# akshilpatel/tile-match-gym

Measured on AMD Instinct MI355X. Metric: env-steps/sec (whole node), 65536×10×10 boards, at 1/2/4/8 MI355X, higher is better.
Workload: dtype int8; 1 GPU; c2: 65536 x 10x10 boards per GPU, 4 colours, no specials, num_moves=30, autoreset, 3 episode-phase blocks offset by 10 steps, the timed window opening on a block's reset step (phases + 4); boards_per_gpu=65536, rows=10, cols=10, colours=4, env_groups_per_gpu=3, phase_blocks=3, policy=uniform, api=raw, graph=False, parallelism=dp1 (independent env shards, no collective)

## Files before the change

### tile-match-gym_amd/csrc/tmg_board.hip

```cpp
#include <hip/hip_runtime.h>
#include <stdint.h>

#include "pcg64.h"

namespace tmg {

#define WSYNC() __syncthreads()

#ifndef TMG_LEAN128_WAVES
#define TMG_LEAN128_WAVES 8
#endif
constexpr int kLean128Waves = TMG_LEAN128_WAVES;
constexpr int kLean128GenericWaves = 7;
constexpr int kGen128Waves = 5;
#ifndef TMG_RESET512_WAVES
#define TMG_RESET512_WAVES 8
#endif
#ifndef TMG_RESET128_WAVES
#define TMG_RESET128_WAVES 8
#endif
constexpr int kReset512Waves = TMG_RESET512_WAVES;
constexpr int kReset128Waves = TMG_RESET128_WAVES;
constexpr int kC5StepWaves = 4;

#define WFENCE() __builtin_amdgcn_fence(__ATOMIC_SEQ_CST, "wavefront")

#ifndef TMG_SMEM_DECL
#define TMG_SMEM_DECL(name) extern __shared__ __align__(16) unsigned char name[]
#endif

enum : int { SP_COOKIE = 1, SP_VLASER = 2, SP_HLASER = 4, SP_BOMB = 8 };
enum : int { M_NORMAL = 0, M_VLASER = 1, M_HLASER = 2, M_BOMB = 3, M_COOKIE = 4 };
enum : int { FL_DONE = 1, FL_COMBO = 2, FL_SHUF = 4, FL_RESET = 8, FL_OVF = 0x40, FL_ERR = 0x80 };
enum : int { TIER_MAIN = 0, TIER_SPILL = 2 };
enum : uint32_t { ST_INTERNAL = 1, ST_OVERFLOW = 2, ST_CALLER = 4 };

constexpr int kMaxShuffles = 1 << 12;

constexpr int kSpillWaves = 16;
struct SpillQ {
    uint32_t count, done;
    unsigned long long total;
    int64_t cap;
    int64_t env[1];
};

#ifndef TMG_COVER
#define TMG_COVER 0
#endif
enum : int {
    CV_SB_LEAN = 0,
    CV_SB_NORMAL,
    CV_SB_LASER,
    CV_SB_PERP_BOMB,
    CV_SB_ROW_BOMB,
    CV_SB_CLOSURE,
    CV_SB_FALLBACK,
    CV_LDS_NORMAL,
    CV_LDS_LASER,
    CV_LDS_BOMB,
    CV_LDS_FALLBACK,
    CV_SERIAL_STEP,
    CV_SERIAL_ACT,
    CV_SERIAL_COOKIE,
    CV_COMBO,
    CV_SPILL,
    CV_SPILL_RUN,
    CV_SHUFFLE,
    CV_REJECT,
    CV_FAST,
    CV_SHUFFLE_GEN,
    CV_REJECT_GEN,
    CV_RP_PASSES,
    CV_RP_PERP,
    CV_RP_VLONG,
    CV_RP_WIDE,
    CV_RP_REJECT,
    CV_COUNT = 32
};
#if TMG_COVER
#define COVER(site)                                                                                     \
    do {                                                                                                \
        if (lane == 0 && P.cover) atomicAdd(P.cover + (site), 1ULL);                                   \
    } while (0)
#define COVER_L0(site)                                                                                  \
    do {                                                                                                \
        if (P.cover) atomicAdd(P.cover + (site), 1ULL);                                                \
    } while (0)
#else
#define COVER(site) ((void)0)
#define COVER_L0(site) ((void)0)
#endif

struct Params {
    int R, C, N, A, W, k, smask, num_moves;
    uint32_t thr;
    uint32_t cmag, cm1mag;
    const uint64_t *jump;
    uint64_t sb_nl[2];
    uint64_t sb_nf[2];
    uint64_t sb_h[2];
    uint64_t sb_z;
    uint64_t sb_in[2], sb_u[2], sb_v[2];
    const uint64_t *sb_rows;
    uint32_t *status;
    void *oh;
    int oh_dtype, oh_ch, oh_nsel;
    uint32_t oh_sel;
    SpillQ *spill;
    void *spill_ws;
    unsigned long long *cover;
    uint8_t *vo_term;
    uint8_t *vo_mask;
    int64_t *vo_left;
    int8_t *vo_final;
    int32_t *vo_obs;
    int sample;
    int32_t pol_t;
    int64_t pol_first;
    uint64_t pol_key;
};

#ifndef TMG_KERNARG_PARAMS
#if defined(__HIP_DEVICE_COMPILE__)
#define TMG_KERNARG_PARAMS(p) (*(const Params *)__builtin_amdgcn_kernarg_segment_ptr())
#else
#define TMG_KERNARG_PARAMS(p) (p)
#endif
#endif

inline void build_sb_rows(int R, int C, uint64_t *tab) {
    for (int r = 0; r < R; r++) {
        uint64_t m[4] = {0, 0, 0, 0};
        for (int p = 0; p < (r + 1) * C && p < 128; p++) {
            if (p >= r * C) m[p & 1] |= 1ULL << (p >> 1);
            m[2 + (p & 1)] |= 1ULL << (p >> 1);
        }
        for (int i = 0; i < 4; i++) tab[r * 4 + i] = m[i];
    }
}

inline Params make_params(int R, int C, int k, int smask, int num_moves, const uint64_t *jump) {
    Params P;
    P.R = R; P.C = C; P.N = R * C;
    P.A = 2 * R * C - R - C;
    P.W = (P.A + 63) / 64;
    P.k = k; P.smask = smask; P.num_moves = num_moves;
    const uint32_t rng = (uint32_t)(k - 1), excl = rng + 1;
    P.thr = rng ? (UINT32_MAX - rng) % excl : 0u;
    P.cmag = ((1u << 20) + (uint32_t)C - 1) / (uint32_t)C;
    P.cm1mag = C > 1 ? ((1u << 20) + (uint32_t)C - 2) / (uint32_t)(C - 1) : 0u;
    P.jump = jump;
    for (int w = 0; w < 2; w++) P.sb_nl[w] = P.sb_nf[w] = P.sb_h[w] = P.sb_in[w] = P.sb_u[w] = P.sb_v[w] = 0;
    P.sb_z = 0;
    P.sb_rows = nullptr;
    P.status = nullptr;
    P.spill = nullptr;
    P.spill_ws = nullptr;
    P.cover = nullptr;
    P.oh = nullptr;
    P.oh_dtype = P.oh_ch = P.oh_nsel = 0;
    P.oh_sel = 0;
    P.vo_term = nullptr;
    P.vo_mask = nullptr;
    P.vo_left = nullptr;
    P.vo_final = nullptr;
    P.vo_obs = nullptr;
    P.sample = 0;
    P.pol_t = 0;
    P.pol_first = 0;
    P.pol_key = 0;
    if (P.N <= 128) {
        for (int p = 0; p < P.N; p++) {
            const int c = p % C, w = p & 1, b = p >> 1;
            P.sb_in[w] |= 1ULL << b;
            if (p >= C) P.sb_u[w] |= 1ULL << b;
            if (p >= 2 * C) P.sb_v[w] |= 1ULL << b;
            if (c <= C - 2) P.sb_nl[w] |= 1ULL << b;
            if (c >= 1) P.sb_nf[w] |= 1ULL << b;
            if (c <= C - 3) P.sb_h[w] |= 1ULL << b;
        }
        const int stride = (C & 1) ? C : C / 2;
        for (int b = 0; b < 64; b += stride) P.sb_z |= 1ULL << b;
    }
    return P;
}

__device__ __forceinline__ int div_c(const Params &P, int x) { return (int)(((uint32_t)x * P.cmag) >> 20); }
__device__ __forceinline__ int div_cm1(const Params &P, int x) { return (int)(((uint32_t)x * P.cm1mag) >> 20); }


__device__ __forceinline__ int64_t wg_env() {
    const int64_t per = gridDim.x >> 3;
    return (int64_t)(blockIdx.x & 7) * per + (blockIdx.x >> 3);
}

enum : int { SC_NACT = 0, SC_NNEW, SC_ERR, SC_NZ, SC_A, SC_B, SC_C, SC_D, SC_COUNT = 16 };

template <int MAXN_>
struct WsCore {
    static constexpr int MAXN = MAXN_;
    static constexpr int NP = MAXN / 64;
    static constexpr int MAXW = (2 * MAXN) / 64 + 2;
    uint64_t effw[MAXW];
    int32_t sc[SC_COUNT];
    static constexpr int PRE = MAXW * 8 + SC_COUNT * 4;
    int8_t lpad[PRE >= 128 ? 1 : 128 - PRE];
    alignas(4) int8_t brd[2 * MAXN];
    uint8_t mark[MAXN];
    alignas(8) int8_t trash[4 * 64];
    union alignas(16) {
        uint32_t draw[MAXN + 128];
        struct { int8_t tmp[2 * MAXN]; int16_t perm[MAXN]; } sh;
    } u;
};

template <int POOL_, int MLINES_, int MQ_, int MM_, int MPOOL_, int MSTK_>
struct ListStore {
    static constexpr int POOL = POOL_;
    static constexpr int MLINES = MLINES_;
    static constexpr int MQ = MQ_;
    static constexpr int MM = MM_;
    static constexpr int MPOOL = MPOOL_;
    static constexpr int MSTK = MSTK_;
    static constexpr int MV = 96;
    int16_t pool[POOL];
    int16_t ls[MLINES], ll[MLINES];
    int16_t q[MQ];
    int16_t mpool[MPOOL];
    int16_t ms[MM], mlen[MM];
    int8_t mname[MM], mcol[MM];
    int16_t fcell[MSTK], fidx[MSTK];
    int8_t ftype[MSTK], faux[MSTK];
    int16_t valid[MV];
    int16_t taken[MM], qpos[MM];
    int8_t qname[MM], qcol[MM];
    int32_t counts[16];
    int16_t pick[4];
};

constexpr int kCap128 = 64;
constexpr int kCap512 = 80;
template <int MAXN, int CAP = (MAXN > 128 ? kCap512 : kCap128)>
using WsSerial = ListStore<4 * CAP + 256, CAP + 64, 2 * CAP + 64, CAP + 32, 4 * CAP + 256, CAP + 8>;

template <int MAXN, int POOLB = 5 * MAXN + 3 * 64 + 64, int LINESB = 2 * MAXN + 2 * 64 + POOLB / 5 + 16>
using WsSerialBig = ListStore<POOLB, LINESB, LINESB, LINESB, POOLB + 3 * LINESB, MAXN + 8>;

template <int MAXN, bool GEN>
struct Ws : WsCore<MAXN> {};
template <int MAXN>
struct Ws<MAXN, true> : WsCore<MAXN> {
    WsSerial<MAXN> s;
};

__device__ __forceinline__ uint32_t umin(uint32_t a, uint32_t b) { return a < b ? a : b; }
__device__ __forceinline__ uint32_t umin3(uint32_t a, uint32_t b, uint32_t c) { return umin(umin(a, b), c); }
__device__ __forceinline__ uint32_t ne(int a, int b) { return (uint32_t)(a ^ b); }

__device__ __forceinline__ int wave_max(int v) {
    const int lo = (int)0x80000000;
    v = max(v, __builtin_amdgcn_update_dpp(lo, v, 0x111, 0xf, 0xf, false));
    v = max(v, __builtin_amdgcn_update_dpp(lo, v, 0x112, 0xf, 0xf, false));
    v = max(v, __builtin_amdgcn_update_dpp(lo, v, 0x114, 0xf, 0xf, false));
    v = max(v, __builtin_amdgcn_update_dpp(lo, v, 0x118, 0xf, 0xf, false));
    v = max(v, __builtin_amdgcn_update_dpp(lo, v, 0x142, 0xa, 0xf, false));
    v = max(v, __builtin_amdgcn_update_dpp(lo, v, 0x143, 0xc, 0xf, false));
    return __builtin_amdgcn_readlane(v, 63);
}

__device__ __forceinline__ int popc_below(uint64_t m) {
    return (int)__builtin_amdgcn_mbcnt_hi((uint32_t)(m >> 32), __builtin_amdgcn_mbcnt_lo((uint32_t)m, 0u));
}
#ifndef TMG_OPAQUE_V
#define TMG_OPAQUE_V(x) asm volatile("" : "+v"(x))
#endif
#ifndef TMG_KEEP_V
#define TMG_KEEP_V(x) asm volatile("" ::"v"(x))
// ... 133 lines not shown
struct Cells {
    uint32_t pk[NP];
    __device__ __forceinline__ int key(int i) const { return (int)(pk[i] & 0x7fffu); }
    __device__ __forceinline__ int r(int i) const { return (int)((pk[i] >> 9) & 63u); }
    __device__ __forceinline__ int c(int i) const { return 255 - (int)((pk[i] >> 1) & 255u); }
    __device__ __forceinline__ uint32_t vbad(int i) const { return (pk[i] >> 15) & 1u; }
    __device__ __forceinline__ uint32_t hbad(int i) const { return (pk[i] >> 16) & 1u; }
};
template <int NP>
__device__ __forceinline__ Cells<NP> make_cells(const Params &P, int lane) {
    Cells<NP> cl;
#pragma unroll
    for (int i = 0; i < NP; i++) {
        const int p = i * 64 + lane;
        const int r = div_c(P, p), c = p - r * P.C;
        const uint32_t vbad = (p < P.N && r >= 2) ? 0u : 1u;
        const uint32_t hbad = (p < P.N && c + 2 < P.C) ? 0u : 1u;
        cl.pk[i] = ((uint32_t)(((r & 63) << 8) | (255 - (c & 255))) << 1) | (vbad << 15) | (hbad << 16);
    }
    return cl;
}

template <class WS>
__device__ __forceinline__ void load_board(const Params &P, WS &w, int lane, const int8_t *src) {
    const int nb = 2 * P.N;
    if ((nb & 3) == 0) {
        const uint32_t *s = reinterpret_cast<const uint32_t *>(src);
        uint32_t *d = reinterpret_cast<uint32_t *>(w.brd);
        for (int i = lane; i < (nb >> 2); i += 64) d[i] = s[i];
    } else {
        for (int i = lane; i < nb; i += 64) w.brd[i] = src[i];
    }
}
template <class WS>
__device__ __forceinline__ void store_board(const Params &P, const WS &w, int lane, int8_t *dst) {
    const int nb = 2 * P.N;
    if ((nb & 3) == 0) {
        uint32_t *d = reinterpret_cast<uint32_t *>(dst);
        const uint32_t *s = reinterpret_cast<const uint32_t *>(w.brd);
        for (int i = lane; i < (nb >> 2); i += 64) d[i] = s[i];
    } else {
        for (int i = lane; i < nb; i += 64) dst[i] = w.brd[i];
    }
}

template <class WS>
__device__ __forceinline__ void store_onehot(const Params &P, const WS &w, int lane, int64_t e) {
    const int N = P.N, k = P.k, ch = P.oh_ch;
    const bool bytes = P.oh_dtype == 1;
    const uint32_t one = P.oh_dtype == 0 ? 0x3f800000u : 1u;
    uint8_t *o8 = reinterpret_cast<uint8_t *>(P.oh) + e * (int64_t)ch * N;
    uint32_t *o32 = reinterpret_cast<uint32_t *>(P.oh) + e * (int64_t)ch * N;
    for (int p = lane; p < N; p += 64) {
        const int x = w.brd[p], y = w.brd[N + p];
        for (int c = 0; c < ch; c++) {
            const bool on = c < k ? x == c + 1 : y == (int)(int8_t)(P.oh_sel >> (8 * (c - k)));
            if (bytes) o8[c * N + p] = on ? 1 : 0;
            else o32[c * N + p] = on ? one : 0u;
        }
    }
}

template <class WS>
__device__ __forceinline__ void store_mask(const Params &P, const WS &w, int lane, int64_t e, bool zero) {
    const int A = P.A;
    uint8_t *m = P.vo_mask + e * (int64_t)A;
    if ((A & 3) == 0) {
        uint32_t *m4 = reinterpret_cast<uint32_t *>(m);
        for (int i = lane; i < (A >> 2); i += 64) {
            const uint32_t b = zero ? 0u : (uint32_t)(w.effw[i >> 4] >> ((4 * i) & 63)) & 0xFu;
            m4[i] = (b * 0x00204081u) & 0x01010101u;
        }
    } else {
        for (int i = lane; i < A; i += 64) m[i] = zero ? (uint8_t)0 : (uint8_t)((w.effw[i >> 6] >> (i & 63)) & 1ULL);
    }
}

template <class WS>
__device__ __forceinline__ void store_obs(const Params &P, const WS &w, int lane, int64_t e) {
    int32_t *o = P.vo_obs + e * 2 * (int64_t)P.N;
    for (int p = lane; p < 2 * P.N; p += 64) o[p] = w.brd[p];
}

__device__ __forceinline__ void store_vo(const Params &P, int64_t e, int flags, int tnew) {
    if (P.vo_term) {
        const uint32_t v = ((flags & FL_DONE) ? 1u : 0u) | ((flags & FL_COMBO) ? 1u << 8 : 0u) |
                           ((flags & FL_SHUF) ? 1u << 16 : 0u) |
                           ((flags & (FL_ERR | FL_OVF)) ? 1u << 24 : 0u);
        reinterpret_cast<uint32_t *>(P.vo_term)[e] = v;
    }
    if (P.vo_left) P.vo_left[e] = (int64_t)(P.num_moves - tnew);
}

__host__ __device__ __forceinline__ uint64_t splitmix64(uint64_t x) {
    x += 0x9E3779B97F4A7C15ULL;
    x = (x ^ (x >> 30)) * 0xBF58476D1CE4E5B9ULL;
    x = (x ^ (x >> 27)) * 0x94D049BB133111EBULL;
    return x ^ (x >> 31);
}
__host__ __device__ __forceinline__ uint64_t policy_draw(uint64_t key, uint64_t gid, int32_t t) {
    const uint64_t base = splitmix64(key * 0xD1B54A32D192ED03ULL + gid);
    return splitmix64(base ^ ((uint64_t)t * 0x9E3779B97F4A7C15ULL)) >> 32;
}

__device__ __forceinline__ int sample_action(const Params &P, uint64_t effrow, int64_t e, int lane) {
#ifndef TMG_DRAW_VALU
#define TMG_DRAW_VALU 0
#endif
#if TMG_DRAW_VALU
    uint64_t gid = (uint64_t)(P.pol_first + e);
    TMG_OPAQUE_V(gid);
    const uint32_t h = (uint32_t)__builtin_amdgcn_readfirstlane((int)(uint32_t)policy_draw(P.pol_key, gid, P.pol_t));
#else
#ifndef TMG_KO
#define TMG_KO 0
#endif
    const uint32_t h = (TMG_KO & 2) ? (uint32_t)(e * 2654435761u) : (uint32_t)policy_draw(P.pol_key, (uint64_t)(P.pol_first + e), P.pol_t);
#endif
    const int W = P.W;
    const int pc = __popcll(effrow);
    int count = 0;
    for (int j = 0; j < W; j++) count += __builtin_amdgcn_readlane(pc, j);
    if (count == 0) return (int)(((uint64_t)h * (uint64_t)P.A) >> 32);
    int r = (int)(((uint64_t)h * (uint64_t)count) >> 32);
    int j = 0;
    for (; j < W - 1; j++) {
        const int c = __builtin_amdgcn_readlane(pc, j);
        if (r < c) break;
        r -= c;
    }
    const uint64_t x = rdlane64(effrow, j);
    const bool hit = ((x >> lane) & 1ULL) && popc_below(x) == r;
    return j * 64 + __ffsll((unsigned long long)__ballot(hit)) - 1;
}

__device__ __forceinline__ int nth_set_bit(uint64_t x, int r) {
    int pos = 0;
#pragma unroll
    for (int sh = 32; sh > 0; sh >>= 1) {
        const int c = __popcll(x & ((1ULL << sh) - 1ULL));
        const bool up = r >= c;
        r -= up ? c : 0;
        x = up ? x >> sh : x;
        pos += up ? sh : 0;
    }
    return pos;
}
__device__ __forceinline__ int32_t draw_row(const uint64_t *m, int W, int A, uint64_t h) {
    int count = 0;
    for (int j = 0; j < W; j++) count += __popcll(m[j]);
    if (count == 0) return (int32_t)((h * (uint64_t)A) >> 32);
    int r = (int)((h * (uint64_t)count) >> 32);
    int j = 0;
    uint64_t x = m[0];
    for (int c = __popcll(x); r >= c && j < W - 1; c = __popcll(x)) {
        r -= c;
        x = m[++j];
    }
    return j * 64 + nth_set_bit(x, r);
}

__device__ __forceinline__ bool eff_exact(const Params &P, const int8_t *brd, int a) {
    const int R = P.R, C = P.C, N = P.N;
    int r1, c1, r2, c2;
    action_coords(R, C, a, r1, c1, r2, c2);
    const int8_t *col = brd, *typ = brd + N;
    const int p = r1 * C + c1, q = r2 * C + c2;
    const int tp = typ[p], tq = typ[q];
    if ((tp != 0 && tp != 1) && (tq != 0 && tq != 1)) return true;
    if (tp < 0 || tq < 0) return true;
    const int cp = col[p], cq = col[q];
    auto CO = [&](int x) -> int { return x == p ? cq : (x == q ? cp : (int)col[x]); };
    auto TY = [&](int x) -> int { return x == p ? tq : (x == q ? tp : (int)typ[x]); };
    int rmin = (r1 < r2 ? r1 : r2) - 2; if (rmin < 0) rmin = 0;
// ... 1462 lines not shown
                if (r < 0) break;
                if (r > 0) { elim += r; iters++; lim = P.R - 1; continue; }
                COVER(CV_SB_FALLBACK);
            }
        }
        Det<MAXN / 64> d;
        const int rs = detect(P, w, lane, cells(), d, lim);
        if (rs < 0) break;
        lim = P.R - 1;
        if (fast) {
            COVER(CV_FAST);
            elim += fast_clear(P, w, lane, cells(), d, rs);
            lim = min(P.R - 1, rs + 2);
        } else {
            if constexpr (GEN && SBNB == 0) {
                uint64_t cols = 0;
                int rows = 0;
                const int r = plain ? simple_step_lds(P, w, lane, d, rs, cols, rows) : 0;
                if (r > 0) {
                    elim += r;
                    gravity(P, w, lane, cols);
                    WSYNC();
                    refill(P, w, lane, J, g, rows);
                    iters++;
                    lim = min(P.R - 1, rs + 2);
                    continue;
                }
                if (plain) COVER(CV_LDS_FALLBACK);
            }
            if constexpr (GEN) {
                int nz = count_colour_nonzero(P, w, lane);
                COVER(CV_SERIAL_STEP);
                if (lane == 0) {
                    w.sc[SC_NZ] = nz;
                    Serial<MAXN, L> S(P, w, *lists);
                    S.build_lines(rs);
                    if (!S.ovf) S.process_lines();
                    if (!S.ovf) S.resolve();
                    w.sc[SC_A] = S.ovf;
                }
                WSYNC();
                ovf |= w.sc[SC_A] != 0;
                elim += count_type_zero(P, w, lane);
            }
        }
        gravity(P, w, lane);
        WSYNC();
        refill(P, w, lane, J, g);
        iters++;
    }
    (void)iters;
    nn = w.sc[SC_NNEW];
    na = w.sc[SC_NACT];
    elim += nn;
    if (ovf) flags |= FL_OVF;
    if (err || w.sc[SC_ERR]) flags |= FL_ERR;
    flags |= ensure_playable(P, w, lane, J, g, cells(), !ovf && !err && !w.sc[SC_ERR]);
    return elim;
}

__device__ __forceinline__ LaneJump load_jump(const Params &P, int lane, const Rng &g) {
    const uint64_t *t = P.jump + lane * 4;
    LaneJump J;
    J.Aj = U128{t[0], t[1]};
    J.Gj = U128{t[2], t[3]};
    J.incG = mul128(U128{g.ilo, g.ihi}, J.Gj);
    return J;
}

__device__ __forceinline__ Rng load_rng(const uint64_t *p) {
    Rng g;
    g.slo = bcast64(p[0]); g.shi = bcast64(p[1]); g.ilo = bcast64(p[2]); g.ihi = bcast64(p[3]); g.h = bcast64(p[4]);
    return g;
}
__device__ __forceinline__ void store_rng(uint64_t *p, const Rng &g, int lane) {
    if (lane == 0) { p[0] = g.slo; p[1] = g.shi; p[2] = g.ilo; p[3] = g.ihi; p[4] = g.h; }
}

#include "tmg_rp.hip"

template <int MAXN, bool GEN, int SBNB, bool CODD, int TIER = TIER_MAIN, class WS = Ws<MAXN, GEN>,
          class L = WsSerial<MAXN>>
__device__ __forceinline__ uint32_t step_env(
    const Params &P, WS &w, int lane, int64_t e, int8_t *__restrict__ board, uint64_t *__restrict__ rng, int32_t *__restrict__ timer,
    const int32_t *__restrict__ actions, int32_t *__restrict__ reward, int32_t *__restrict__ n_new,
    int32_t *__restrict__ n_act, uint8_t *__restrict__ flags_out, uint64_t *__restrict__ eff, int trust_eff,
    int autoreset, L *lists) {
    const int N = P.N, W = P.W;
    constexpr bool INLINE_GEN = !GEN && MAXN == 128;
    const bool same = autoreset == 1 || autoreset == 2;
    const bool regen_inline = autoreset == 1 || autoreset == 3;
    int a = __builtin_amdgcn_readfirstlane(actions[e]);
    const int t0 = __builtin_amdgcn_readfirstlane(timer[e]);
    const uint64_t effrow = lane < W ? eff[e * W + lane] : 0ULL;
    TMG_KEEP_V(effrow);
    if (P.sample) {
        a = __builtin_amdgcn_readfirstlane(sample_action(P, effrow, e, lane));
        if (lane == 0) const_cast<int32_t *>(actions)[e] = a;
    }
#ifndef TMG_QEXIT
#define TMG_QEXIT 1
#endif
    if (TMG_QEXIT && trust_eff && t0 < P.num_moves - 1 && (unsigned)a < (unsigned)P.A) {
        if (!((rdlane64(effrow, a >> 6) >> (a & 63)) & 1ULL)) {
            if (lane == 0) {
                uint64_t ve = (uint64_t)e;
                TMG_OPAQUE_V(ve);
                timer[ve] = t0 + 1;
                reward[ve] = 0; n_new[ve] = 0; n_act[ve] = 0;
                flags_out[ve] = (uint8_t)0;
                if (P.vo_term) reinterpret_cast<uint32_t *>(P.vo_term)[ve] = 0u;
                if (P.vo_left) P.vo_left[ve] = (int64_t)(P.num_moves - 1 - t0);
            }
            return 0;
        }
    }
    bool pend = false;
    if (t0 >= P.num_moves || a < 0 || a >= P.A) {
        pend = autoreset >= 3 && t0 >= P.num_moves;
    }
    if (!pend && (t0 >= P.num_moves || a < 0 || a >= P.A)) {
        if (lane == 0) {
            reward[e] = 0; n_new[e] = 0; n_act[e] = 0; flags_out[e] = FL_ERR;
            store_vo(P, e, FL_ERR, t0);
        }
        if ((P.oh || P.vo_obs) && !trust_eff) {
            load_board(P, w, lane, board + e * 2 * N);
            WSYNC();
            if (P.oh) store_onehot(P, w, lane, e);
            if (P.vo_obs) store_obs(P, w, lane, e);
        }
        return ST_CALLER;
    }
    int8_t *gb = board + e * 2 * N;
    uint64_t *ge = eff + e * W;
    const int t1 = t0 + 1;
    const bool done = !pend && t1 == P.num_moves;
    const bool regen = pend || (done && same);
    int flags = done ? FL_DONE : 0;
    bool effective = false;
    if (trust_eff && !pend) {
        effective = (rdlane64(effrow, a >> 6) >> (a & 63)) & 1ULL;
    }
    if (trust_eff && !effective && !(regen && regen_inline)) {
        const bool defer = regen;
        if (done && !same) {
            for (int i = lane; i < W; i += 64) ge[i] = 0ULL;
            if (P.vo_mask) store_mask(P, w, lane, e, true);
        }
        if (done && same && P.vo_final) {
            const int nbw = ((2 * N) & 3) == 0 ? (2 * N) >> 2 : 0;
            const uint32_t *src = reinterpret_cast<const uint32_t *>(gb);
            uint32_t *dst = reinterpret_cast<uint32_t *>(P.vo_final + e * 2 * N);
            for (int i = lane; i < nbw; i += 64) dst[i] = src[i];
            for (int i = 4 * nbw + lane; i < 2 * N; i += 64) P.vo_final[e * 2 * N + i] = gb[i];
        }
        if (lane == 0) {
            const int tn = defer ? 0 : t1;
            timer[e] = tn; reward[e] = 0; n_new[e] = 0; n_act[e] = 0;
            flags_out[e] = (uint8_t)(flags | (defer ? FL_RESET : 0));
            store_vo(P, e, flags, tn);
        }
        return 0;
    }
    int r1, c1, r2, c2;
    action_coords(P.R, P.C, a, r1, c1, r2, c2);
    const int p1 = r1 * P.C + c1, p2 = r2 * P.C + c2;

    const int nbw = (2 * N) >> 2;
    const bool bwhole = ((2 * N) & 3) == 0 && nbw <= 64;
    const uint32_t bw = bwhole ? reinterpret_cast<const uint32_t *>(gb)[lane < nbw ? lane : 0] : 0u;
    const uint64_t *rp = rng + e * 5;
    const uint64_t q0 = rp[0], q1 = rp[1], q2 = rp[2], q3 = rp[3], q4 = rp[4];
    constexpr bool RP = SBNB > 0 && !GEN;
    bool rowp = false;
    if constexpr (RP) rowp = rp_shape(P);
    const uint64_t *jt = P.jump + (rowp ? bp_out(lane) : lane) * 4;
    const uint64_t j0 = jt[0], j1 = jt[1], j2 = jt[2], j3 = jt[3];
    if (bwhole) {
        if (lane < nbw) reinterpret_cast<uint32_t *>(w.brd)[lane] = bw;
    } else {
        load_board(P, w, lane, gb);
    }
    if constexpr (GEN) {
        for (int p = lane; p < N; p += 64) w.mark[p] = 0;
    }
    if constexpr (TIER == TIER_SPILL) COVER(CV_SPILL_RUN);
    WSYNC();
    if constexpr (!GEN) {
        bool ok = true;
        for (int p = lane; p < N; p += 64) ok &= w.brd[N + p] == 1;
        if (__ballot(!ok) != 0ULL) {
            if (lane == 0) {
                reward[e] = 0; n_new[e] = 0; n_act[e] = 0; flags_out[e] = FL_ERR;
                store_vo(P, e, FL_ERR, t0);
            }
            return ST_INTERNAL;
        }
    }
    if (!trust_eff && !pend) {
        bool ex = lane == 0 ? eff_exact(P, w.brd, a) : false;
        effective = __ballot(ex) != 0ULL;
    }
    Rng g;
    g.slo = bcast64(q0); g.shi = bcast64(q1); g.ilo = bcast64(q2); g.ihi = bcast64(q3); g.h = bcast64(q4);
    LaneJump J;
    J.Aj = U128{j0, j1};
    J.Gj = U128{j2, j3};
    J.incG = mul128(U128{g.ilo, g.ihi}, J.Gj);
    const Cells<MAXN / 64> cl = make_cells<MAXN / 64>(P, lane);
    int elim = 0, nn = 0, na = 0;
    bool changed = false;
    if (effective) {
        if constexpr (RP) {
            if (rowp) elim = rp_move<SBNB, CODD>(P, w, lane, J, g, cl, p1, p2, flags);
            else elim = sb_move<SBNB, CODD>(P, w, lane, J, g, cl, p1, p2, flags, e);
        } else elim = board_move<MAXN, GEN, SBNB, CODD, TIER>(P, w, lane, J, g, cl, p1, p2, flags, nn, na, e, lists,
                                                             trust_eff != 0);
        changed = true;
        if constexpr (GEN) {
            if (flags & FL_OVF) {
                if constexpr (TIER == TIER_MAIN) {
                    if (queue_env(P.spill, lane, e)) { COVER(CV_SPILL); return 0; }
                }
                flags = (flags & ~FL_OVF) | FL_ERR;
            }
        }
    }
    int tnew = t1;
    if (regen) {
        if (done && P.vo_final) store_board(P, w, lane, P.vo_final + e * 2 * N);
        if constexpr (INLINE_GEN) {
            if (regen_inline) {
                int fg = -1;
                if constexpr (SBNB > 0) {
                    if (P.C <= 32) fg = bp_generate<SBNB>(P, w, lane, g);
                    if (fg < 0) {
                        if (rowp) J = load_jump(P, lane, g);
                        fg = sb_generate_exact<SBNB, CODD>(P, w, lane, J, g, cl);
                    }
                } else {
                    fg = generate_board(P, w, lane, J, g, cl);
                }
                flags |= fg;
                changed = true;
            }
        }
        tnew = 0;
        flags |= FL_RESET;
    }
    if (changed) {
        store_board(P, w, lane, gb);
        store_rng(rng + e * 5, g, lane);
    }
    if (P.oh && (changed || !trust_eff)) store_onehot(P, w, lane, e);
    if (P.vo_obs && (changed || !trust_eff)) store_obs(P, w, lane, e);
    if (done && !same) {
        for (int i = lane; i < W; i += 64) ge[i] = 0ULL;
        if (P.vo_mask) store_mask(P, w, lane, e, true);
    } else if (changed) {
        for (int i = lane; i < W; i += 64) ge[i] = w.effw[i];
        if (P.vo_mask) store_mask(P, w, lane, e, false);
    } else if (!trust_eff) {
        scan_effective(P, w, lane, cl, false);
        WSYNC();
        for (int i = lane; i < W; i += 64) ge[i] = w.effw[i];
        if (P.vo_mask) store_mask(P, w, lane, e, false);
    }
    if (lane == 0) {
        timer[e] = tnew;
        reward[e] = elim;
        n_new[e] = nn;
        n_act[e] = na;
        flags_out[e] = (uint8_t)flags;
        store_vo(P, e, flags, tnew);
    }
    return ((flags & FL_ERR) ? ST_INTERNAL : 0u) | ((flags & FL_OVF) ? ST_OVERFLOW : 0u);
}

#if defined(__clang__)
#define TMG_ASSUME(x) __builtin_assume(x)
#else
#define TMG_ASSUME(x) do { if (!(x)) __builtin_unreachable(); } while (0)
#endif
constexpr int shape_fix(int R, int C, int k, int smask) { return (R << 24) | (C << 16) | (k << 8) | smask; }
constexpr int kNoFix = 0;
constexpr int kFixAnySpecials = 255;
constexpr int kFixC2 = shape_fix(10, 10, 4, 0);
constexpr int kFixC3 = shape_fix(10, 10, 4, SP_VLASER | SP_HLASER | SP_BOMB);
constexpr int kFixC5 = shape_fix(20, 20, 6, SP_COOKIE | SP_VLASER | SP_HLASER | SP_BOMB);
constexpr int kFixReset10 = shape_fix(10, 10, 4, kFixAnySpecials);
constexpr int kFixReset20 = shape_fix(20, 20, 6, kFixAnySpecials);
__host__ __device__ constexpr uint64_t fix_mask(int R, int C, int w, int what) {
    uint64_t m = 0;
    for (int p = 0; p < R * C && p < 128; p++) {
        const int c = p % C;
        if ((p & 1) != w) continue;
        const bool on = what == 0 ? true : what == 1 ? p >= C : what == 2 ? p >= 2 * C : what == 3 ? c <= C - 2
                      : what == 4 ? c >= 1 : c <= C - 3;
        if (on) m |= 1ULL << (p >> 1);
    }
    return m;
}
template <int FIX>
__device__ __forceinline__ void assume_shape(const Params &P) {
    if constexpr (FIX != kNoFix) {
        constexpr struct { int R, C, K, smask; } F{FIX >> 24, (FIX >> 16) & 255, (FIX >> 8) & 255, FIX & 255};
        TMG_ASSUME(P.R == F.R);
        TMG_ASSUME(P.C == F.C);
        TMG_ASSUME(P.N == F.R * F.C);
        TMG_ASSUME(P.A == 2 * F.R * F.C - F.R - F.C);
        TMG_ASSUME(P.W == (2 * F.R * F.C - F.R - F.C + 63) / 64);
        TMG_ASSUME(P.k == F.K);
        if constexpr (F.smask != kFixAnySpecials) TMG_ASSUME(P.smask == F.smask);
        TMG_ASSUME(P.thr == (F.K > 1 ? (0xffffffffu - (uint32_t)(F.K - 1)) % (uint32_t)F.K : 0u));
        TMG_ASSUME(P.cmag == ((1u << 20) + (uint32_t)F.C - 1) / (uint32_t)F.C);
        TMG_ASSUME(P.cm1mag == ((1u << 20) + (uint32_t)F.C - 2) / (uint32_t)(F.C - 1));
        if constexpr (F.R * F.C <= 128) {
#define TMG_ASSUME_MASK(field, what)                                          \
    {                                                                         \
        constexpr uint64_t m0 = fix_mask(F.R, F.C, 0, what), m1 = fix_mask(F.R, F.C, 1, what); \
        TMG_ASSUME(P.field[0] == m0);                                   \
        TMG_ASSUME(P.field[1] == m1);                                   \
    }
            TMG_ASSUME_MASK(sb_in, 0)
            TMG_ASSUME_MASK(sb_u, 1)
            TMG_ASSUME_MASK(sb_v, 2)
            TMG_ASSUME_MASK(sb_nl, 3)
            TMG_ASSUME_MASK(sb_nf, 4)
            TMG_ASSUME_MASK(sb_h, 5)
#undef TMG_ASSUME_MASK
        }
    }
}

template <int MAXN, bool GEN, int SBNB = 0, bool CODD = false, int FIX = kNoFix>
__global__ __launch_bounds__(64, MAXN == 128 ? (GEN ? kGen128Waves : (FIX != kNoFix ? kLean128Waves : kLean128GenericWaves))
                                            : (FIX == kFixC5 ? kC5StepWaves : 1)) void step_kernel(
    Params P_, int64_t n, int8_t *__restrict__ board, uint64_t *__restrict__ rng, int32_t *__restrict__ timer,
    const int32_t *__restrict__ actions, int32_t *__restrict__ reward, int32_t *__restrict__ n_new,
    int32_t *__restrict__ n_act, uint8_t *__restrict__ flags_out, uint64_t *__restrict__ eff, int trust_eff,
    int autoreset) {
    TMG_SMEM_DECL(smem);
    using WS = Ws<MAXN, GEN>;
    const Params &P = TMG_KERNARG_PARAMS(P_);
    assume_shape<FIX>(P);
    const int lane = threadIdx.x & 63;
    WS &w = *reinterpret_cast<WS *>(smem);
    const int64_t e = wg_env();
    if (e >= n) return;
    WsSerial<MAXN> *lists = nullptr;
    if constexpr (GEN) lists = &w.s;
    const uint32_t st = step_env<MAXN, GEN, SBNB, CODD, TIER_MAIN, WS, WsSerial<MAXN>>(
        P, w, lane, e, board, rng, timer, actions, reward, n_new, n_act, flags_out, eff, trust_eff, autoreset, lists);
    note_status(P, lane, st);
}

template <int MAXN>
__global__ __launch_bounds__(64, 8) void spill_kernel(
    Params P, int64_t n, int8_t *__restrict__ board, uint64_t *__restrict__ rng, int32_t *__restrict__ timer,
    const int32_t *__restrict__ actions, int32_t *__restrict__ reward, int32_t *__restrict__ n_new,
    int32_t *__restrict__ n_act, uint8_t *__restrict__ flags_out, uint64_t *__restrict__ eff, int trust_eff,
    int autoreset) {
    TMG_SMEM_DECL(smem);
    using WS = Ws<MAXN, false>;
    const int lane = threadIdx.x & 63;
    WS &w = *reinterpret_cast<WS *>(smem);
    SpillQ *q = P.spill;
    WsSerialBig<MAXN> *lists = reinterpret_cast<WsSerialBig<MAXN> *>(P.spill_ws) + blockIdx.x;
    const int64_t queued = (int64_t)(uint32_t)__builtin_amdgcn_readfirstlane((int)q->count);
    const int cnt = (int)(queued < q->cap ? queued : q->cap);
    int done = 0;
    for (int i = (int)blockIdx.x; i < cnt; i += (int)gridDim.x) {
        const int64_t e = (int64_t)bcast64((uint64_t)q->env[i]);
        if (e < 0 || e >= n) continue;
        WSYNC();
        const uint32_t st = step_env<MAXN, true, 0, false, TIER_SPILL, WS, WsSerialBig<MAXN>>(
            P, w, lane, e, board, rng, timer, actions, reward, n_new, n_act, flags_out, eff, trust_eff, autoreset, lists);
        note_status(P, lane, st);
        done++;
    }
    if (lane == 0) {
        if (done) atomicAdd(&q->total, (unsigned long long)done);
        __threadfence();
        if (atomicAdd(&q->done, 1u) == gridDim.x - 1) { q->count = 0u; q->done = 0u; }
    }
}

template <int MAXN, int SBNB, bool CODD, class WS>
__device__ __forceinline__ void reset_env(const Params &P, WS &w, int lane, int64_t e, int8_t *__restrict__ board,
                                          uint64_t *__restrict__ rng, int32_t *__restrict__ timer,
                                          uint64_t *__restrict__ eff) {
    const int N = P.N, W = P.W;
    Rng g = load_rng(rng + e * 5);
    const Cells<MAXN / 64> cl = make_cells<MAXN / 64>(P, lane);
    int fl = -1;
    if constexpr (SBNB > 0) {
        if (P.C <= 32) fl = bp_generate<SBNB, (MAXN > 128)>(P, w, lane, g);
    }
    if (fl < 0) {
        const LaneJump J = load_jump(P, lane, g);
        if constexpr (MAXN == 128 && SBNB > 0) fl = sb_generate_exact<SBNB, CODD>(P, w, lane, J, g, cl);
        else fl = generate_board(P, w, lane, J, g, cl);
    }
    note_status(P, lane, fl ? ST_INTERNAL : 0u);
    store_board(P, w, lane, board + e * 2 * N);
    store_rng(rng + e * 5, g, lane);
    if (P.oh) store_onehot(P, w, lane, e);
    if (P.vo_obs) store_obs(P, w, lane, e);
    for (int i = lane; i < W; i += 64) eff[e * W + i] = w.effw[i];
    if (P.vo_mask) store_mask(P, w, lane, e, false);
    if (lane == 0) {
        timer[e] = 0;
        if (P.vo_left) P.vo_left[e] = P.num_moves;
    }
}

template <int MAXN, int SBNB = 0, bool CODD = false, int FIX = kNoFix>
__global__ __launch_bounds__(64, MAXN > 128 ? kReset512Waves : (FIX != kNoFix ? kReset128Waves : 1)) void reset_kernel(Params P_, int64_t n, int8_t *__restrict__ board,
                                                             uint64_t *__restrict__ rng, int32_t *__restrict__ timer,
                                                             uint64_t *__restrict__ eff,
                                                             const uint8_t *__restrict__ env_mask, int mask_bits,
                                                             int epw) {
    TMG_SMEM_DECL(smem);
    using WS = Ws<MAXN, false>;
    const Params &P = TMG_KERNARG_PARAMS(P_);
    assume_shape<FIX>(P);
    const int lane = threadIdx.x & 63;
    WS &w = *reinterpret_cast<WS *>(smem);
    const int64_t e0 = wg_env() * epw;
    if (e0 >= n) return;
    const int64_t el = e0 + lane;
    uint64_t todo = __ballot(lane < epw && el < n && (!env_mask || (env_mask[el] & mask_bits)));
    while (todo) {
        const int k = __builtin_ctzll(todo);
        todo &= todo - 1;
        reset_env<MAXN, SBNB, CODD>(P, w, loop_lane(lane), e0 + k, board, rng, timer, eff);
        WSYNC();
    }
}

template <int MAXN>
__global__ __launch_bounds__(64) void effective_kernel(Params P, int64_t n, const int8_t *__restrict__ board,
                                                                 uint64_t *__restrict__ eff) {
    TMG_SMEM_DECL(smem);
    using WS = Ws<MAXN, false>;
    const int lane = threadIdx.x & 63;
    WS &w = *reinterpret_cast<WS *>(smem);
    const int64_t e = wg_env();
    if (e >= n) return;
    load_board(P, w, lane, board + e * 2 * P.N);
    WSYNC();
    const Cells<MAXN / 64> cl = make_cells<MAXN / 64>(P, lane);
    scan_effective(P, w, lane, cl, false);
    WSYNC();
    for (int i = lane; i < P.W; i += 64) eff[e * P.W + i] = w.effw[i];
}

}
```

### tile-match-gym_amd/csrc/tmg_kernels.hip

```cpp
#include <hip/hip_runtime.h>

#include "tmg_board.hip"
#include "tmg_dispatch.h"
#include "tmg_launch.h"
#if TMG_TU == 1
#include "tmg_lane.h"
#endif
#if TMG_TU == 6
#include "tmg_aux.hip"
#endif

#ifndef TMG_TU
#error "compile tmg_kernels.hip with -DTMG_TU=1..7"
#endif

namespace tmg {

namespace {

struct StepLaunch {
    dim3 grid;
    hipStream_t s;
    const Params &P;
    const StepArgs &a;
    template <int MAXN, bool GEN, int NB, bool CODD, int FIX>
    void step() {
        const size_t lds = sizeof(Ws<MAXN, GEN>);
        hipLaunchKernelGGL((step_kernel<MAXN, GEN, NB, CODD, FIX>), grid, dim3(64), lds, s, P, a.n, a.board, a.rng,
                           a.timer, a.actions, a.reward, a.n_new, a.n_act, a.flags, a.eff, a.trust_eff, a.autoreset);
    }
};

template <int MAXN>
void spill_one(hipStream_t s, const Params &P, const StepArgs &a) {
    const size_t lds = sizeof(Ws<MAXN, false>);
    hipLaunchKernelGGL((spill_kernel<MAXN>), dim3(kSpillWaves), dim3(64), lds, s, P, a.n, a.board, a.rng, a.timer,
                       a.actions, a.reward, a.n_new, a.n_act, a.flags, a.eff, a.trust_eff, a.autoreset);
}

struct ResetLaunch {
    dim3 grid;
    hipStream_t s;
    const Params &P;
    int64_t n;
    int8_t *board;
    uint64_t *rng;
    int32_t *timer;
    uint64_t *eff;
    const uint8_t *env_mask;
    int mask_bits, epw;
    template <int MAXN, int NB, bool CODD, int FIX>
    void reset() {
        const size_t lds = sizeof(Ws<MAXN, false>);
        hipLaunchKernelGGL((reset_kernel<MAXN, NB, CODD, FIX>), grid, dim3(64), lds, s, P, n, board, rng, timer, eff,
                           env_mask, mask_bits, epw);
    }
};

struct EffectiveLaunch {
    dim3 grid;
    hipStream_t s;
    const Params &P;
    int64_t n;
    const int8_t *board;
    uint64_t *eff;
    template <int MAXN>
    void effective() {
        hipLaunchKernelGGL(effective_kernel<MAXN>, grid, dim3(64), sizeof(Ws<MAXN, false>), s, P, n, board, eff);
    }
};

}

#if TMG_TU == 1
#ifndef TMG_LANE_WPE
#define TMG_LANE_WPE 0
#endif
#ifndef TMG_LANE_LDS
#define TMG_LANE_LDS 0
#endif
template <int R, int C, int K, int EPW>
__global__ __launch_bounds__(64)
#if TMG_LANE_WPE > 0
__attribute__((amdgpu_waves_per_eu(TMG_LANE_WPE, TMG_LANE_WPE)))
#endif
void lane_step_kernel(Params P_, int64_t n, int8_t *__restrict__ board, uint64_t *__restrict__ rng,
                      int32_t *__restrict__ timer, int32_t *__restrict__ actions, int32_t *__restrict__ reward,
                      int32_t *__restrict__ n_new, int32_t *__restrict__ n_act, uint8_t *__restrict__ flags,
                      uint64_t *__restrict__ eff, int autoreset) {
    __shared__ uint8_t scratch[EPW * kLaneScratch + TMG_LANE_LDS];
    const Params &P = TMG_KERNARG_PARAMS(P_);
    const int lane = threadIdx.x & 63;
    const int64_t e = wg_env() * EPW + lane;
    if (lane >= EPW || e >= n) return;
    const lane::StepIO io{board, rng, timer, actions, reward, n_new, n_act, flags, eff,
                          P.num_moves, autoreset, P.sample, P.pol_key, P.pol_first, P.pol_t};
    const uint32_t st = lane::step_env<lane::Board<R, C, K>>(io, e, scratch + lane * kLaneScratch);
    if (st & lane::LS_INTERNAL) P.status[0] = 1u;
    if (st & lane::LS_CALLER) P.status[2] = 1u;
}

template <int K, int EPW>
void lane_one(hipStream_t s, const Params &P, const StepArgs &a) {
    const dim3 grid = env_grid((a.n + EPW - 1) / EPW);
    int32_t *act = const_cast<int32_t *>(a.actions);
    hipLaunchKernelGGL((lane_step_kernel<10, 10, K, EPW>), grid, dim3(64), 0, s, P, a.n, a.board, a.rng, a.timer,
                       act, a.reward, a.n_new, a.n_act, a.flags, a.eff, a.autoreset);
}

void launch_step_lane(hipStream_t s, const Params &P, const StepArgs &a) {
    const bool small = a.n < kLaneSmallEnvs;
// ... 86 lines not shown
```

Before: 1.185 billion env-steps/s.

## Load hot step kernel arguments as two contiguous scalar blocks from kernarg

Reorders the Params struct so the fields the step kernel uses most (output pointers, jump table, A/W, num_moves, option bits, grid size) sit at its tail, next to the kernel's scalar arguments. For the c2 fixed shape, the kernel reads those 128 bytes with two s_load_dwordx16 instructions in inline asm instead of many scattered scalar loads, and it tests precomputed option bits instead of checking several pointers. The aim is shorter kernel-entry latency and fewer SGPR loads per short wave. In exchange it depends on struct layout (guarded by static_asserts) and hand-written asm that assumes the kernarg layout.

```diff
diff --git a/tile-match-gym_amd/csrc/tmg_board.hip b/tile-match-gym_amd/csrc/tmg_board.hip
--- a/tile-match-gym_amd/csrc/tmg_board.hip
+++ b/tile-match-gym_amd/csrc/tmg_board.hip
@@ -1,5 +1,6 @@
 #include <hip/hip_runtime.h>
 #include <stdint.h>
+#include <cstddef>
 
 #include "pcg64.h"
 
@@ -93,33 +94,72 @@
 #endif
 
 struct Params {
-    int R, C, N, A, W, k, smask, num_moves;
+    int R, C, N, A, W, k, smask;
     uint32_t thr;
     uint32_t cmag, cm1mag;
-    const uint64_t *jump;
     uint64_t sb_nl[2];
     uint64_t sb_nf[2];
     uint64_t sb_h[2];
     uint64_t sb_z;
     uint64_t sb_in[2], sb_u[2], sb_v[2];
     const uint64_t *sb_rows;
+    SpillQ *spill;
+    void *spill_ws;
+    unsigned long long *cover;
+    int64_t pol_first;
+    uint64_t pol_key;
     uint32_t *status;
     void *oh;
     int oh_dtype, oh_ch, oh_nsel;
     uint32_t oh_sel;
-    SpillQ *spill;
-    void *spill_ws;
-    unsigned long long *cover;
-    uint8_t *vo_term;
     uint8_t *vo_mask;
-    int64_t *vo_left;
     int8_t *vo_final;
     int32_t *vo_obs;
+    int32_t pol_t;
     int sample;
-    int32_t pol_t;
-    int64_t pol_first;
-    uint64_t pol_key;
+    uint8_t *vo_term;
+    int64_t *vo_left;
+    const uint64_t *jump;
+    uint32_t aw;
+    int num_moves;
+    uint32_t opts;
+    uint32_t grid;
 };
+
+enum : uint32_t { OPT_SAMPLE = 1, OPT_OH = 2, OPT_VO_MASK = 4, OPT_VO_FINAL = 8, OPT_VO_OBS = 16 };
+__host__ __device__ inline uint32_t step_opts(const Params &P) {
+    return (P.sample ? OPT_SAMPLE : 0u) | (P.oh ? OPT_OH : 0u) | (P.vo_mask ? OPT_VO_MASK : 0u) |
+           (P.vo_final ? OPT_VO_FINAL : 0u) | (P.vo_obs ? OPT_VO_OBS : 0u);
+}
+
+#define TMG_HOT_TAIL_FIELDS \
+    uint8_t *vo_term;       \
+    int64_t *vo_left;       \
+    const uint64_t *jump;   \
+    uint32_t aw;            \
+    int num_moves;          \
+    uint32_t opts;          \
+    uint32_t grid;
+struct HotTail {
+    TMG_HOT_TAIL_FIELDS
+};
+static_assert(sizeof(Params) % 8 == 0 && offsetof(Params, vo_term) + sizeof(HotTail) == sizeof(Params) &&
+                  offsetof(Params, grid) - offsetof(Params, vo_term) == offsetof(HotTail, grid),
+              "HotTail mirrors the tail of Params");
+
+struct StepHot {
+    TMG_HOT_TAIL_FIELDS
+    int64_t n;
+    int8_t *board;
+    uint64_t *rng;
+    int32_t *timer;
+    const int32_t *actions;
+    int32_t *reward, *n_new, *n_act;
+    uint8_t *flags_out;
+    uint64_t *eff;
+    int trust_eff, autoreset;
+};
+static_assert(sizeof(StepHot) == 128 && offsetof(StepHot, n) == sizeof(HotTail), "StepHot is two 64-byte loads");
 
 #ifndef TMG_KERNARG_PARAMS
 #if defined(__HIP_DEVICE_COMPILE__)
@@ -129,6 +169,40 @@
 #endif
 #endif
 
+#ifndef TMG_ENTRY_BLOCK
+#if defined(__HIP_DEVICE_COMPILE__)
+typedef uint32_t kv16 __attribute__((ext_vector_type(16)));
+template <class T>
+__device__ __forceinline__ T *kernarg_global(T *p) {
+    return (T *)(__attribute__((address_space(1))) T *)(uintptr_t)p;
+}
+#define TMG_GLOBAL(p) (kernarg_global(p))
+template <class H, int OFF>
+__device__ __forceinline__ H kernarg_block() {
+    static_assert(sizeof(H) == 128, "two 64-byte loads");
+    const uint64_t ka = (uint64_t)__builtin_amdgcn_kernarg_segment_ptr();
+    H h;
+    struct { kv16 a, b; } v;
+    asm("s_load_dwordx16 %0, %2, %3\n\ts_load_dwordx16 %1, %2, %4\n\ts_waitcnt lgkmcnt(0)"
+        : "=&s"(v.a), "=&s"(v.b)
+        : "s"(ka), "n"(OFF), "n"(OFF + 64));
+    __builtin_memcpy(&h, &v, sizeof(H));
+    return h;
+}
+#define TMG_ENTRY_BLOCK(H, p, ...) (kernarg_block<H, offsetof(Params, vo_term)>())
+#define TMG_LAUNCH_OPTS(p) ((p).opts)
+#else
+#define TMG_ENTRY_BLOCK(H, p, ...) \
+    (H{(p).vo_term, (p).vo_left, (p).jump, (p).aw, (p).num_moves, step_opts(p), (p).grid, __VA_ARGS__})
+#endif
+#endif
+#ifndef TMG_LAUNCH_OPTS
+#define TMG_LAUNCH_OPTS(p) (step_opts(p))
+#endif
+#ifndef TMG_GLOBAL
+#define TMG_GLOBAL(p) (p)
+#endif
+
 inline void build_sb_rows(int R, int C, uint64_t *tab) {
     for (int r = 0; r < R; r++) {
         uint64_t m[4] = {0, 0, 0, 0};
@@ -145,6 +219,7 @@
     P.R = R; P.C = C; P.N = R * C;
     P.A = 2 * R * C - R - C;
     P.W = (P.A + 63) / 64;
+    P.aw = (uint32_t)P.A | ((uint32_t)P.W << 16);
     P.k = k; P.smask = smask; P.num_moves = num_moves;
     const uint32_t rng = (uint32_t)(k - 1), excl = rng + 1;
     P.thr = rng ? (UINT32_MAX - rng) % excl : 0u;
@@ -168,8 +243,10 @@
     P.vo_obs = nullptr;
     P.sample = 0;
     P.pol_t = 0;
+    P.opts = 0;
     P.pol_first = 0;
     P.pol_key = 0;
+    P.grid = 0;
     if (P.N <= 128) {
         for (int p = 0; p < P.N; p++) {
             const int c = p % C, w = p & 1, b = p >> 1;
@@ -190,10 +267,11 @@
 __device__ __forceinline__ int div_cm1(const Params &P, int x) { return (int)(((uint32_t)x * P.cm1mag) >> 20); }
 
 
-__device__ __forceinline__ int64_t wg_env() {
-    const int64_t per = gridDim.x >> 3;
+__device__ __forceinline__ int64_t wg_env(uint32_t grid) {
+    const int64_t per = grid >> 3;
     return (int64_t)(blockIdx.x & 7) * per + (blockIdx.x >> 3);
 }
+__device__ __forceinline__ int64_t wg_env() { return wg_env(gridDim.x); }
 
 enum : int { SC_NACT = 0, SC_NNEW, SC_ERR, SC_NZ, SC_A, SC_B, SC_C, SC_D, SC_COUNT = 16 };
 
@@ -493,14 +571,17 @@
     for (int p = lane; p < 2 * P.N; p += 64) o[p] = w.brd[p];
 }
 
-__device__ __forceinline__ void store_vo(const Params &P, int64_t e, int flags, int tnew) {
-    if (P.vo_term) {
+template <class PH>
+__device__ __forceinline__ void store_vo(const PH &P, int64_t e, int flags, int tnew) {
+    uint8_t *const vo_term = TMG_GLOBAL(P.vo_term);
+    int64_t *const vo_left = TMG_GLOBAL(P.vo_left);
+    if (vo_term) {
         const uint32_t v = ((flags & FL_DONE) ? 1u : 0u) | ((flags & FL_COMBO) ? 1u << 8 : 0u) |
                            ((flags & FL_SHUF) ? 1u << 16 : 0u) |
                            ((flags & (FL_ERR | FL_OVF)) ? 1u << 24 : 0u);
-        reinterpret_cast<uint32_t *>(P.vo_term)[e] = v;
-    }
-    if (P.vo_left) P.vo_left[e] = (int64_t)(P.num_moves - tnew);
+        reinterpret_cast<uint32_t *>(vo_term)[e] = v;
+    }
+    if (vo_left) vo_left[e] = (int64_t)(P.num_moves - tnew);
 }
 
 __host__ __device__ __forceinline__ uint64_t splitmix64(uint64_t x) {
@@ -2129,11 +2210,12 @@
 template <int MAXN, bool GEN, int SBNB, bool CODD, int TIER = TIER_MAIN, class WS = Ws<MAXN, GEN>,
           class L = WsSerial<MAXN>>
 __device__ __forceinline__ uint32_t step_env(
-    const Params &P, WS &w, int lane, int64_t e, int8_t *__restrict__ board, uint64_t *__restrict__ rng, int32_t *__restrict__ timer,
-    const int32_t *__restrict__ actions, int32_t *__restrict__ reward, int32_t *__restrict__ n_new,
-    int32_t *__restrict__ n_act, uint8_t *__restrict__ flags_out, uint64_t *__restrict__ eff, int trust_eff,
-    int autoreset, L *lists) {
-    const int N = P.N, W = P.W;
+    const Params &P, const StepHot &H, WS &w, int lane, int64_t e, int8_t *__restrict__ board, uint64_t *__restrict__ rng,
+    int32_t *__restrict__ timer, const int32_t *__restrict__ actions, int32_t *__restrict__ reward,
+    int32_t *__restrict__ n_new, int32_t *__restrict__ n_act, uint8_t *__restrict__ flags_out,
+    uint64_t *__restrict__ eff, L *lists) {
+    const int trust_eff = H.trust_eff, autoreset = H.autoreset;
+    const int N = P.N, HA = (int)(H.aw & 0xffffu), W = (int)(H.aw >> 16);
     constexpr bool INLINE_GEN = !GEN && MAXN == 128;
     const bool same = autoreset == 1 || autoreset == 2;
     const bool regen_inline = autoreset == 1 || autoreset == 3;
@@ -2141,14 +2223,14 @@
     const int t0 = __builtin_amdgcn_readfirstlane(timer[e]);
     const uint64_t effrow = lane < W ? eff[e * W + lane] : 0ULL;
     TMG_KEEP_V(effrow);
-    if (P.sample) {
+    if (H.opts & OPT_SAMPLE) {
         a = __builtin_amdgcn_readfirstlane(sample_action(P, effrow, e, lane));
         if (lane == 0) const_cast<int32_t *>(actions)[e] = a;
     }
 #ifndef TMG_QEXIT
 #define TMG_QEXIT 1
 #endif
-    if (TMG_QEXIT && trust_eff && t0 < P.num_moves - 1 && (unsigned)a < (unsigned)P.A) {
+    if (TMG_QEXIT && trust_eff && t0 < H.num_moves - 1 && (unsigned)a < (unsigned)HA) {
         if (!((rdlane64(effrow, a >> 6) >> (a & 63)) & 1ULL)) {
             if (lane == 0) {
                 uint64_t ve = (uint64_t)e;
@@ -2156,33 +2238,33 @@
                 timer[ve] = t0 + 1;
                 reward[ve] = 0; n_new[ve] = 0; n_act[ve] = 0;
                 flags_out[ve] = (uint8_t)0;
-                if (P.vo_term) reinterpret_cast<uint32_t *>(P.vo_term)[ve] = 0u;
-                if (P.vo_left) P.vo_left[ve] = (int64_t)(P.num_moves - 1 - t0);
+                if (H.vo_term) reinterpret_cast<uint32_t *>(TMG_GLOBAL(H.vo_term))[ve] = 0u;
+                if (H.vo_left) TMG_GLOBAL(H.vo_left)[ve] = (int64_t)(H.num_moves - 1 - t0);
             }
             return 0;
         }
     }
     bool pend = false;
-    if (t0 >= P.num_moves || a < 0 || a >= P.A) {
-        pend = autoreset >= 3 && t0 >= P.num_moves;
-    }
-    if (!pend && (t0 >= P.num_moves || a < 0 || a >= P.A)) {
+    if (t0 >= H.num_moves || a < 0 || a >= HA) {
+        pend = autoreset >= 3 && t0 >= H.num_moves;
+    }
+    if (!pend && (t0 >= H.num_moves || a < 0 || a >= HA)) {
         if (lane == 0) {
             reward[e] = 0; n_new[e] = 0; n_act[e] = 0; flags_out[e] = FL_ERR;
-            store_vo(P, e, FL_ERR, t0);
-        }
-        if ((P.oh || P.vo_obs) && !trust_eff) {
+            store_vo(H, e, FL_ERR, t0);
+        }
+        if ((H.opts & (OPT_OH | OPT_VO_OBS)) && !trust_eff) {
             load_board(P, w, lane, board + e * 2 * N);
             WSYNC();
-            if (P.oh) store_onehot(P, w, lane, e);
-            if (P.vo_obs) store_obs(P, w, lane, e);
+            if (H.opts & OPT_OH) store_onehot(P, w, lane, e);
+            if (H.opts & OPT_VO_OBS) store_obs(P, w, lane, e);
         }
         return ST_CALLER;
     }
     int8_t *gb = board + e * 2 * N;
     uint64_t *ge = eff + e * W;
     const int t1 = t0 + 1;
-    const bool done = !pend && t1 == P.num_moves;
+    const bool done = !pend && t1 == H.num_moves;
     const bool regen = pend || (done && same);
     int flags = done ? FL_DONE : 0;
     bool effective = false;
@@ -2193,9 +2275,9 @@
         const bool defer = regen;
         if (done && !same) {
             for (int i = lane; i < W; i += 64) ge[i] = 0ULL;
-            if (P.vo_mask) store_mask(P, w, lane, e, true);
-        }
-        if (done && same && P.vo_final) {
+            if (H.opts & OPT_VO_MASK) store_mask(P, w, lane, e, true);
+        }
+        if (done && same && (H.opts & OPT_VO_FINAL)) {
             const int nbw = ((2 * N) & 3) == 0 ? (2 * N) >> 2 : 0;
             const uint32_t *src = reinterpret_cast<const uint32_t *>(gb);
             uint32_t *dst = reinterpret_cast<uint32_t *>(P.vo_final + e * 2 * N);
@@ -2206,7 +2288,7 @@
             const int tn = defer ? 0 : t1;
             timer[e] = tn; reward[e] = 0; n_new[e] = 0; n_act[e] = 0;
             flags_out[e] = (uint8_t)(flags | (defer ? FL_RESET : 0));
-            store_vo(P, e, flags, tn);
+            store_vo(H, e, flags, tn);
         }
         return 0;
     }
@@ -2222,7 +2304,7 @@
     constexpr bool RP = SBNB > 0 && !GEN;
     bool rowp = false;
     if constexpr (RP) rowp = rp_shape(P);
-    const uint64_t *jt = P.jump + (rowp ? bp_out(lane) : lane) * 4;
+    const uint64_t *jt = TMG_GLOBAL(H.jump) + (rowp ? bp_out(lane) : lane) * 4;
     const uint64_t j0 = jt[0], j1 = jt[1], j2 = jt[2], j3 = jt[3];
     if (bwhole) {
         if (lane < nbw) reinterpret_cast<uint32_t *>(w.brd)[lane] = bw;
@@ -2240,7 +2322,7 @@
         if (__ballot(!ok) != 0ULL) {
             if (lane == 0) {
                 reward[e] = 0; n_new[e] = 0; n_act[e] = 0; flags_out[e] = FL_ERR;
-                store_vo(P, e, FL_ERR, t0);
+                store_vo(H, e, FL_ERR, t0);
             }
             return ST_INTERNAL;
         }
@@ -2276,7 +2358,7 @@
     }
     int tnew = t1;
     if (regen) {
-        if (done && P.vo_final) store_board(P, w, lane, P.vo_final + e * 2 * N);
+        if (done && (H.opts & OPT_VO_FINAL)) store_board(P, w, lane, P.vo_final + e * 2 * N);
         if constexpr (INLINE_GEN) {
             if (regen_inline) {
                 int fg = -1;
@@ -2300,19 +2382,19 @@
         store_board(P, w, lane, gb);
         store_rng(rng + e * 5, g, lane);
     }
-    if (P.oh && (changed || !trust_eff)) store_onehot(P, w, lane, e);
-    if (P.vo_obs && (changed || !trust_eff)) store_obs(P, w, lane, e);
+    if ((H.opts & OPT_OH) && (changed || !trust_eff)) store_onehot(P, w, lane, e);
+    if ((H.opts & OPT_VO_OBS) && (changed || !trust_eff)) store_obs(P, w, lane, e);
     if (done && !same) {
         for (int i = lane; i < W; i += 64) ge[i] = 0ULL;
-        if (P.vo_mask) store_mask(P, w, lane, e, true);
+        if (H.opts & OPT_VO_MASK) store_mask(P, w, lane, e, true);
     } else if (changed) {
         for (int i = lane; i < W; i += 64) ge[i] = w.effw[i];
-        if (P.vo_mask) store_mask(P, w, lane, e, false);
+        if (H.opts & OPT_VO_MASK) store_mask(P, w, lane, e, false);
     } else if (!trust_eff) {
         scan_effective(P, w, lane, cl, false);
         WSYNC();
         for (int i = lane; i < W; i += 64) ge[i] = w.effw[i];
-        if (P.vo_mask) store_mask(P, w, lane, e, false);
+        if (H.opts & OPT_VO_MASK) store_mask(P, w, lane, e, false);
     }
     if (lane == 0) {
         timer[e] = tnew;
@@ -2320,7 +2402,7 @@
         n_new[e] = nn;
         n_act[e] = na;
         flags_out[e] = (uint8_t)flags;
-        store_vo(P, e, flags, tnew);
+        store_vo(H, e, flags, tnew);
     }
     return ((flags & FL_ERR) ? ST_INTERNAL : 0u) | ((flags & FL_OVF) ? ST_OVERFLOW : 0u);
 }
@@ -2381,6 +2463,18 @@
     }
 }
 
+template <int FIX>
+constexpr bool kEntryBlock = FIX == kFixC2;
+
+template <int FIX, class H>
+__device__ __forceinline__ void assume_shape_hot(const H &h) {
+    if constexpr (FIX != kNoFix) {
+        constexpr struct { int R, C; } F{FIX >> 24, (FIX >> 16) & 255};
+        constexpr uint32_t A = 2 * F.R * F.C - F.R - F.C;
+        TMG_ASSUME(h.aw == (A | ((A + 63) / 64) << 16));
+    }
+}
+
 template <int MAXN, bool GEN, int SBNB = 0, bool CODD = false, int FIX = kNoFix>
 __global__ __launch_bounds__(64, MAXN == 128 ? (GEN ? kGen128Waves : (FIX != kNoFix ? kLean128Waves : kLean128GenericWaves))
                                             : (FIX == kFixC5 ? kC5StepWaves : 1)) void step_kernel(
@@ -2392,14 +2486,24 @@
     using WS = Ws<MAXN, GEN>;
     const Params &P = TMG_KERNARG_PARAMS(P_);
     assume_shape<FIX>(P);
+    StepHot H;
+    if constexpr (kEntryBlock<FIX>) {
+        H = TMG_ENTRY_BLOCK(StepHot, P_, n, board, rng, timer, actions, reward, n_new, n_act, flags_out, eff, trust_eff,
+                            autoreset);
+    } else {
+        H = StepHot{P.vo_term, P.vo_left, P.jump, P.aw, P.num_moves, TMG_LAUNCH_OPTS(P), gridDim.x, n, board, rng, timer,
+                    actions, reward, n_new, n_act, flags_out, eff, trust_eff, autoreset};
+    }
+    assume_shape_hot<FIX>(H);
     const int lane = threadIdx.x & 63;
     WS &w = *reinterpret_cast<WS *>(smem);
-    const int64_t e = wg_env();
-    if (e >= n) return;
+    const int64_t e = wg_env(H.grid);
+    if (e >= H.n) return;
     WsSerial<MAXN> *lists = nullptr;
     if constexpr (GEN) lists = &w.s;
     const uint32_t st = step_env<MAXN, GEN, SBNB, CODD, TIER_MAIN, WS, WsSerial<MAXN>>(
-        P, w, lane, e, board, rng, timer, actions, reward, n_new, n_act, flags_out, eff, trust_eff, autoreset, lists);
+        P, H, w, lane, e, TMG_GLOBAL(H.board), TMG_GLOBAL(H.rng), TMG_GLOBAL(H.timer), TMG_GLOBAL(H.actions),
+        TMG_GLOBAL(H.reward), TMG_GLOBAL(H.n_new), TMG_GLOBAL(H.n_act), TMG_GLOBAL(H.flags_out), TMG_GLOBAL(H.eff), lists);
     note_status(P, lane, st);
 }
 
@@ -2413,6 +2517,8 @@
     using WS = Ws<MAXN, false>;
     const int lane = threadIdx.x & 63;
     WS &w = *reinterpret_cast<WS *>(smem);
+    const StepHot H{P.vo_term, P.vo_left, P.jump, P.aw, P.num_moves, step_opts(P), gridDim.x, n, board, rng, timer, actions,
+                    reward, n_new, n_act, flags_out, eff, trust_eff, autoreset};
     SpillQ *q = P.spill;
     WsSerialBig<MAXN> *lists = reinterpret_cast<WsSerialBig<MAXN> *>(P.spill_ws) + blockIdx.x;
     const int64_t queued = (int64_t)(uint32_t)__builtin_amdgcn_readfirstlane((int)q->count);
@@ -2423,7 +2529,7 @@
         if (e < 0 || e >= n) continue;
         WSYNC();
         const uint32_t st = step_env<MAXN, true, 0, false, TIER_SPILL, WS, WsSerialBig<MAXN>>(
-            P, w, lane, e, board, rng, timer, actions, reward, n_new, n_act, flags_out, eff, trust_eff, autoreset, lists);
+            P, H, w, lane, e, board, rng, timer, actions, reward, n_new, n_act, flags_out, eff, lists);
         note_status(P, lane, st);
         done++;
     }
diff --git a/tile-match-gym_amd/csrc/tmg_kernels.hip b/tile-match-gym_amd/csrc/tmg_kernels.hip
--- a/tile-match-gym_amd/csrc/tmg_kernels.hip
+++ b/tile-match-gym_amd/csrc/tmg_kernels.hip
@@ -26,7 +26,10 @@
     template <int MAXN, bool GEN, int NB, bool CODD, int FIX>
     void step() {
         const size_t lds = sizeof(Ws<MAXN, GEN>);
-        hipLaunchKernelGGL((step_kernel<MAXN, GEN, NB, CODD, FIX>), grid, dim3(64), lds, s, P, a.n, a.board, a.rng,
+        Params Q = P;
+        Q.grid = grid.x;
+        Q.opts = step_opts(P);
+        hipLaunchKernelGGL((step_kernel<MAXN, GEN, NB, CODD, FIX>), grid, dim3(64), lds, s, Q, a.n, a.board, a.rng,
                            a.timer, a.actions, a.reward, a.n_new, a.n_act, a.flags, a.eff, a.trust_eff, a.autoreset);
     }
 };
```

Result: no change. 1.189 billion env-steps/s, median of 6 (+0.3%).
